# ctb/khmer

Hardware: NVIDIA B200
Metric: kmers_per_sec_countgraph_k20_N4 (higher is better)
Workload: dtype u8

## Files before the change

### include/kmgpu.h

```cpp
#ifndef KMGPU_H
#define KMGPU_H

#include <stddef.h>
#include <stdint.h>

#ifdef __cplusplus
extern "C" {
#endif

#define KMGPU_ABI_VERSION 2

enum { KMGPU_BYTE = 0, KMGPU_NIBBLE = 1, KMGPU_BIT = 2 };
enum { KMGPU_TWOBIT = 0, KMGPU_MURMUR = 1 };

#define KMGPU_CLEAN 1u

enum {
    KMGPU_OK = 0,
    KMGPU_EINVAL = 1,
    KMGPU_ENODEV = 2,
    KMGPU_ECUDA = 3,
    KMGPU_ENOMEM = 4,
    KMGPU_ENONACGT = 5,
    KMGPU_ESHAPE = 6,
// ... 95 lines not shown
int kmgpu_ipc_export(kmgpu_t* h, uint8_t* handles );
int kmgpu_ipc_attach(kmgpu_t* h, int rank, int world, const uint8_t* all_handles );
int kmgpu_ipc_detach(kmgpu_t* h);
int kmgpu_reduce_scatter_peers(kmgpu_t* h);
int kmgpu_all_gather_peers(kmgpu_t* h);
int kmgpu_reduce_replicas(kmgpu_t** replicas, int n);
int kmgpu_attach_replicas(kmgpu_t** replicas, int n);
int kmgpu_slice_range(uint64_t n_words, int world, int rank, uint64_t* w0, uint64_t* w1);

int kmgpu_first_touch_log(kmgpu_t* h, int on);
int kmgpu_first_touch_resolve(kmgpu_t* h, uint64_t* n_new_out, uint64_t* n_local_out, uint64_t* hist);

typedef struct kmgpu_shard kmgpu_shard_t;
#define KMGPU_SHARD_IPC_HANDLES 5
#define KMGPU_MAX_WORLD 16
int kmgpu_shard_create(int storage, int hash, int ksize, int n_tables, const uint64_t* full_sizes, int device,
                       int rank, int world, uint64_t max_positions_per_route, kmgpu_shard_t** out);
int kmgpu_shard_destroy(kmgpu_shard_t* s);
kmgpu_t* kmgpu_shard_local(kmgpu_shard_t* s);
int kmgpu_shard_slice(kmgpu_shard_t* s, int table, uint64_t* lo, uint64_t* hi);
int kmgpu_shard_stats(kmgpu_shard_t* s, uint64_t* n_occupied_local, uint64_t* n_unique_share, uint64_t* store_bytes);
int kmgpu_shard_ipc_export(kmgpu_shard_t* s, uint8_t* handles);
int kmgpu_shard_ipc_attach(kmgpu_shard_t* s, const uint8_t* all_handles);
int kmgpu_shard_attach_local(kmgpu_shard_t** all, int n);
int kmgpu_shard_route(kmgpu_shard_t* s, const char* seqs, const uint64_t* offsets, uint64_t n_reads, uint32_t flags,
                      uint64_t* n_kmers_out);
int kmgpu_shard_offsets(kmgpu_shard_t* s);
int kmgpu_shard_push(kmgpu_shard_t* s);
int kmgpu_shard_apply(kmgpu_shard_t* s);
int kmgpu_shard_count_new(kmgpu_shard_t* s, uint64_t* n_new_out);

int kmgpu_profile_reset(kmgpu_t* h);
int kmgpu_profile_get(kmgpu_t* h, double* ingest_kernel_ms, uint64_t* ingest_launches, uint64_t* all_launches);
int kmgpu_sync(kmgpu_t* h);
int kmgpu_timer_start(kmgpu_t* h);
int kmgpu_timer_stop(kmgpu_t* h, double* ms);

typedef struct kmgpu_hll kmgpu_hll_t;
int kmgpu_hll_create(int device, int ksize, int n_counters_log2, kmgpu_hll_t** out);
int kmgpu_hll_destroy(kmgpu_hll_t* c);
int kmgpu_hll_consume(kmgpu_hll_t* c, const char* seqs, const uint64_t* offsets, uint64_t n_reads, uint32_t flags, uint64_t* n_kmers_out);
int kmgpu_hll_get_registers(kmgpu_hll_t* c, uint8_t* out);
int kmgpu_hll_merge_registers(kmgpu_hll_t* c, const uint8_t* in, int replace);

#ifdef __cplusplus
}
#endif
#endif
```

### khmer_b200/cabi.py

```python
import ctypes as C
import os

import numpy as np

HERE = os.path.dirname(os.path.abspath(__file__))
LIB_PATH = os.path.join(HERE, "libkmgpu.so")

BYTE, NIBBLE, BIT = 0, 1, 2
TWOBIT, MURMUR = 0, 1
CLEAN = 1

u8p = C.POINTER(C.c_uint8)
u16p = C.POINTER(C.c_uint16)
u32p = C.POINTER(C.c_uint32)
u64p = C.POINTER(C.c_uint64)
f32p = C.POINTER(C.c_float)

SYMBOLS = [
    "kmgpu_last_error", "kmgpu_abi_version", "kmgpu_device_count", "kmgpu_create", "kmgpu_destroy",
    "kmgpu_set_use_bigcount", "kmgpu_get_use_bigcount", "kmgpu_consume_reads", "kmgpu_consume_packed",
    "kmgpu_batch_create", "kmgpu_batch_destroy", "kmgpu_batch_info", "kmgpu_consume_batch", "kmgpu_batch_read_medians", "kmgpu_add_hashes",
    "kmgpu_get_counts", "kmgpu_kmer_counts", "kmgpu_kmer_hashes", "kmgpu_read_medians", "kmgpu_median_at_least",
    "kmgpu_abundance_distribution", "kmgpu_trim_batch", "kmgpu_normalize_batch", "kmgpu_consume_reads_new", "kmgpu_first_touch_log",
    "kmgpu_first_touch_resolve", "kmgpu_stats", "kmgpu_set_stats", "kmgpu_shape", "kmgpu_set_ksize",
    "kmgpu_table_nbytes", "kmgpu_download_table", "kmgpu_upload_table", "kmgpu_bigcount_size",
    "kmgpu_bigcount_export", "kmgpu_bigcount_import", "kmgpu_merge", "kmgpu_recount_occupied", "kmgpu_ipc_export",
    "kmgpu_ipc_attach", "kmgpu_ipc_detach", "kmgpu_reduce_scatter_peers", "kmgpu_all_gather_peers",
    "kmgpu_reduce_replicas", "kmgpu_attach_replicas", "kmgpu_profile_reset", "kmgpu_profile_get", "kmgpu_sync", "kmgpu_reset",
    "kmgpu_timer_start", "kmgpu_timer_stop", "kmgpu_slice_range", "kmgpu_alloc_pinned", "kmgpu_free_pinned",
    "kmgpu_shard_create", "kmgpu_shard_destroy", "kmgpu_shard_local", "kmgpu_shard_slice", "kmgpu_shard_ipc_export",
    "kmgpu_shard_ipc_attach", "kmgpu_shard_attach_local", "kmgpu_shard_route", "kmgpu_shard_offsets", "kmgpu_shard_push", "kmgpu_shard_apply",
    "kmgpu_shard_count_new", "kmgpu_shard_stats", "kmgpu_hll_create", "kmgpu_hll_destroy", "kmgpu_hll_consume",
    "kmgpu_hll_get_registers", "kmgpu_hll_merge_registers",
]


class Band(C.Structure):
    _fields_ = [("lo", C.c_uint64), ("hi", C.c_uint64)]


class Mask(C.Structure):
    _fields_ = [("mask", C.c_void_p), ("threshold", C.c_uint32), ("consume_masked", C.c_int)]


class KmgpuError(RuntimeError):
    def __init__(self, code, msg):
        super().__init__("kmgpu error %d: %s" % (code, msg))
        self.code = code
        self.msg = msg


_lib = None


def lib():
    global _lib
    if _lib is None:
        if not os.path.exists(LIB_PATH):
            raise ImportError("%s is missing: build it with `python -c 'import __graft_entry__ as g; g.build()'` "
                              "(nvcc, sm_100a). There is no CPU fallback." % LIB_PATH)
        L = C.CDLL(LIB_PATH)
# ... 25 lines not shown
                                         C.c_void_p, C.c_void_p, C.c_void_p]
        L.kmgpu_median_at_least.argtypes = [C.c_void_p, C.c_void_p, C.c_void_p, C.c_uint64, C.c_uint32, C.c_uint32,
                                            C.c_void_p]
        L.kmgpu_abundance_distribution.argtypes = [C.c_void_p, C.c_void_p, C.c_void_p, C.c_void_p, C.c_uint64,
                                                   C.c_uint32, C.c_void_p]
        L.kmgpu_trim_batch.argtypes = [C.c_void_p, C.c_void_p, C.c_void_p, C.c_uint64, C.c_uint32, C.c_uint32, C.c_int, C.c_void_p]
        L.kmgpu_normalize_batch.argtypes = [C.c_void_p, C.c_void_p, C.c_void_p, C.c_uint64, C.c_uint32, C.c_void_p, C.c_uint32,
                                            C.c_void_p, u64p, u64p]
        L.kmgpu_consume_reads_new.argtypes = [C.c_void_p, C.c_void_p, C.c_void_p, C.c_uint64, C.c_uint32, C.c_void_p, u64p, u64p]
        L.kmgpu_first_touch_log.argtypes = [C.c_void_p, C.c_int]
        L.kmgpu_first_touch_resolve.argtypes = [C.c_void_p, u64p, u64p, C.c_void_p]
        L.kmgpu_stats.argtypes = [C.c_void_p, u64p, u64p]
        L.kmgpu_set_stats.argtypes = [C.c_void_p, C.c_uint64, C.c_uint64]
        L.kmgpu_shape.argtypes = [C.c_void_p, C.POINTER(C.c_int), C.POINTER(C.c_int), C.POINTER(C.c_int),
                                  C.POINTER(C.c_int), u64p]
        L.kmgpu_set_ksize.argtypes = [C.c_void_p, C.c_int]
        L.kmgpu_table_nbytes.argtypes = [C.c_void_p, C.c_int, u64p]
        L.kmgpu_download_table.argtypes = [C.c_void_p, C.c_int, C.c_void_p, C.c_uint64, C.c_uint64]
        L.kmgpu_upload_table.argtypes = [C.c_void_p, C.c_int, C.c_void_p, C.c_uint64, C.c_uint64]
        L.kmgpu_bigcount_size.argtypes = [C.c_void_p, u64p]
        L.kmgpu_bigcount_export.argtypes = [C.c_void_p, C.c_void_p, C.c_void_p, C.c_uint64]
        L.kmgpu_bigcount_import.argtypes = [C.c_void_p, C.c_void_p, C.c_void_p, C.c_uint64]
        L.kmgpu_merge.argtypes = [C.c_void_p, C.c_void_p]
        L.kmgpu_recount_occupied.argtypes = [C.c_void_p]
        L.kmgpu_ipc_export.argtypes = [C.c_void_p, C.c_void_p]
        L.kmgpu_ipc_attach.argtypes = [C.c_void_p, C.c_int, C.c_int, C.c_void_p]
        L.kmgpu_ipc_detach.argtypes = [C.c_void_p]
        L.kmgpu_reduce_scatter_peers.argtypes = [C.c_void_p]
        L.kmgpu_all_gather_peers.argtypes = [C.c_void_p]
        L.kmgpu_reduce_replicas.argtypes = [C.POINTER(C.c_void_p), C.c_int]
        L.kmgpu_attach_replicas.argtypes = [C.POINTER(C.c_void_p), C.c_int]
        L.kmgpu_profile_reset.argtypes = [C.c_void_p]
        L.kmgpu_profile_get.argtypes = [C.c_void_p, C.POINTER(C.c_double), u64p, u64p]
        L.kmgpu_sync.argtypes = [C.c_void_p]
        L.kmgpu_reset.argtypes = [C.c_void_p]
        L.kmgpu_timer_start.argtypes = [C.c_void_p]
        L.kmgpu_timer_stop.argtypes = [C.c_void_p, C.POINTER(C.c_double)]
        L.kmgpu_device_count.argtypes = [C.POINTER(C.c_int)]
        L.kmgpu_slice_range.argtypes = [C.c_uint64, C.c_int, C.c_int, u64p, u64p]
        L.kmgpu_shard_create.argtypes = [C.c_int, C.c_int, C.c_int, C.c_int, u64p, C.c_int, C.c_int, C.c_int, C.c_uint64,
                                         C.POINTER(C.c_void_p)]
        L.kmgpu_shard_destroy.argtypes = [C.c_void_p]
        L.kmgpu_shard_local.restype = C.c_void_p
        L.kmgpu_shard_local.argtypes = [C.c_void_p]
        L.kmgpu_shard_slice.argtypes = [C.c_void_p, C.c_int, u64p, u64p]
        L.kmgpu_shard_ipc_export.argtypes = [C.c_void_p, C.c_void_p]
        L.kmgpu_shard_ipc_attach.argtypes = [C.c_void_p, C.c_void_p]
        L.kmgpu_shard_attach_local.argtypes = [C.POINTER(C.c_void_p), C.c_int]
        L.kmgpu_shard_route.argtypes = [C.c_void_p, C.c_void_p, C.c_void_p, C.c_uint64, C.c_uint32, u64p]
        L.kmgpu_shard_apply.argtypes = [C.c_void_p]
        L.kmgpu_shard_offsets.argtypes = [C.c_void_p]
        L.kmgpu_shard_push.argtypes = [C.c_void_p]
        L.kmgpu_shard_count_new.argtypes = [C.c_void_p, u64p]
        L.kmgpu_shard_stats.argtypes = [C.c_void_p, u64p, u64p, u64p]
        _lib = L
    return _lib


def check(rc):
    if rc != 0:
        raise KmgpuError(rc, lib().kmgpu_last_error().decode(errors="replace"))


def device_count():
    n = C.c_int()
    rc = lib().kmgpu_device_count(C.byref(n))
# ... 291 lines not shown

    def merge(self, other):
        check(lib().kmgpu_merge(self.h, other.h))

    def recount_occupied(self):
        check(lib().kmgpu_recount_occupied(self.h))

    def ipc_export(self):
        out = np.zeros(64 * len(self.sizes), dtype=np.uint8)
        check(lib().kmgpu_ipc_export(self.h, _ptr(out)))
        return out

    def ipc_attach(self, rank, world, all_handles):
        all_handles = np.ascontiguousarray(all_handles, dtype=np.uint8)
        check(lib().kmgpu_ipc_attach(self.h, rank, world, _ptr(all_handles)))

    def ipc_detach(self):
        check(lib().kmgpu_ipc_detach(self.h))

    def reduce_scatter_peers(self):
        check(lib().kmgpu_reduce_scatter_peers(self.h))

    def all_gather_peers(self):
        check(lib().kmgpu_all_gather_peers(self.h))

    def profile_reset(self):
        check(lib().kmgpu_profile_reset(self.h))

    def profile_get(self):
        ms, a, b = C.c_double(), C.c_uint64(), C.c_uint64()
        check(lib().kmgpu_profile_get(self.h, C.byref(ms), C.byref(a), C.byref(b)))
        return ms.value, a.value, b.value

    def sync(self):
        check(lib().kmgpu_sync(self.h))

    def reset(self):
        check(lib().kmgpu_reset(self.h))

    def timer_start(self):
        check(lib().kmgpu_timer_start(self.h))

    def timer_stop(self):
        ms = C.c_double()
        check(lib().kmgpu_timer_stop(self.h, C.byref(ms)))
        return ms.value


SHARD_IPC_HANDLES = 5


class Shard:

    def __init__(self, storage, hashkind, ksize, full_sizes, rank, world, device=0, max_positions=8 << 20):
        self.full_sizes = [int(x) for x in full_sizes]
        arr = (C.c_uint64 * len(self.full_sizes))(*self.full_sizes)
        self.h = C.c_void_p()
        self.storage, self.rank, self.world, self.max_positions = storage, rank, world, max_positions
        check(lib().kmgpu_shard_create(storage, hashkind, ksize, len(self.full_sizes), arr, device, rank, world, max_positions,
                                       C.byref(self.h)))
        self.local = Sketch.__new__(Sketch)
        self.local.h = C.c_void_p(lib().kmgpu_shard_local(self.h))
        self.local.sizes = [max(hi - lo, 1) for lo, hi in (self.slice(i) for i in range(len(self.full_sizes)))]
        self.local.storage, self.local.hashkind, self.local.ksize = storage, hashkind, ksize
        self.local.close = lambda: None

# ... 84 lines not shown
```

### khmer_b200/csrc/kmgpu_api.cu

```cuda
#include <algorithm>
#include <cstdarg>
#include <cstdio>
#include <cstdlib>
#include <cstring>
#include <chrono>
#include <functional>
#include <mutex>
#include <string>
#include <unordered_map>
#include <vector>

#include "../../include/kmgpu.h"
#include "kmgpu_kernels.cuh"
#include "kmgpu_group.cuh"

using namespace kmgpu;

static thread_local std::string g_err;

static int fail(int code, const char* fmt, ...)
{
    char buf[1024];
    va_list ap;
    va_start(ap, fmt);
// ... 1016 lines not shown
    h->all_launches += 1;
    CK(cudaGetLastError());
    CK(cudaMemcpyAsync(h->h_evout.p, h->d_evout.p, n_distinct * sizeof(EvOut), cudaMemcpyDeviceToHost, st));
    CK(cudaStreamSynchronize(st));
    std::vector<EvOut> evs(h->h_evout.p, h->h_evout.p + n_distinct);
    std::sort(evs.begin(), evs.end(), [](const EvOut& a, const EvOut& b) { return a.first < b.first; });
    for (const EvOut& e : evs) big_events(h, e.hash, e.count);
    return KMGPU_OK;
}

static bool plan_buckets(const kmgpu_sketch* h, uint32_t n_pos, BucketLayout* L)
{
    if (!env_u64("KMGPU_BUCKETS", 1)) return false;
    memset(L, 0, sizeof *L);
    L->n_tables = h->nt;
    uint64_t cap = 0, total = 0;
    for (int i = 0; i < h->nt; i++) {
        if (h->sizes[i] > 0xFFFFFFFEull - 128) return false;
        uint64_t nb = (h->sizes[i] + BKT_BINS - 1) / BKT_BINS;
        if (nb > (uint64_t)BKT_MAX_BUCKETS) return false;
        L->first[i] = (uint32_t)total;
        total += nb;
        uint64_t expect = nb == 1 ? n_pos : (uint64_t)((double)n_pos * BKT_BINS / (double)h->sizes[i]) + 1;
        cap = std::max(cap, expect + expect / 4 + 2048);
    }
    L->first[h->nt] = (uint32_t)total;
    cap = std::min<uint64_t>(cap, (uint64_t)n_pos);
    if (uint64_t forced = env_u64("KMGPU_BUCKET_CAP", 0)) cap = forced;
    if (cap > 65535 || cap == 0) return false;
    L->cap = (uint32_t)cap;
    return true;
}

template <int KIND>
static void launch_apply(unsigned g, cudaStream_t st, const SketchDev& S, const BucketLayout& L, const unsigned long long* rec, const uint32_t* cur,
                         uint32_t* newbits, uint64_t* binlist, unsigned long long list_cap, Ctrl* ctrl, int want_cross, const SatBits& sb)
{
    k_apply<KIND><<<g, 1024, BKT_APPLY_SMEM, st>>>(S, L, rec, cur, newbits, binlist, list_cap, ctrl, want_cross, sb);
}

typedef std::function<int()> Between;

#include "kmgpu_group_host.inc"

static int ingest_chunk_delta(kmgpu_sketch* h, const std::vector<DeltaPass>& passes, int src, HashCfg H, const std::vector<Part>& parts, const Pred& P,
                              bool pred, const SketchDev* M, ChunkResult* res, const Between& between)
{
    cudaStream_t st = h->stream;
    uint32_t n_pos = 0;
    for (const Part& pt : parts) n_pos = std::max(n_pos, pt.pos_off + pt.in.n_pos);
    const uint64_t stride = ((uint64_t)n_pos + 7) & ~7ull;
    CKR(h->d_bins.ensure((size_t)h->nt * stride));
    uint64_t total_bins = 0, max_span = 0;
    for (int i = 0; i < h->nt; i++) total_bins += h->sizes[i];
    for (const DeltaPass& p : passes) max_span = std::max<uint64_t>(max_span, p.hi - p.lo);
    const uint64_t list_cap = std::max<uint64_t>(1, std::min<uint64_t>((uint64_t)h->nt * n_pos, total_bins));
    CKR(h->d_binlist.ensure(list_cap));
    size_t need_lanes = h->kind == BIT ? ((max_span + 127) / 128) * 8 + 8 : ((max_span + 7) & ~7ull) + 8;
    if (h->d_delta.cap < need_lanes) h->delta_zeroed = 0;
    CKR(h->d_delta.ensure(need_lanes));
    if (h->delta_zeroed < h->d_delta.cap) {
        CK(cudaMemsetAsync(h->d_delta.p, 0, h->d_delta.cap * 2, st));
        h->delta_zeroed = h->d_delta.cap;
    }
    CK(cudaMemsetAsync(h->d_ctrl, 0, sizeof(Ctrl), st));
    CK(cudaEventRecord(h->ev0, st));
    const int want_cross = h->kind == BYTE && h->use_bigcount;
    if (want_cross && !h->satbits_valid) {
        for (int i = 0; i < h->nt; i++) {
            uint64_t groups = (h->sizes[i] + 7) / 8;
            CKR(h->d_satbits[i].ensure(groups));
            k_build_satbits<<<(unsigned)std::min<uint64_t>((groups + 255) / 256, 148 * 16), 256, 0, st>>>(h->dev.tables[i], groups, h->d_satbits[i].p);
            h->all_launches += 1;
        }
        h->satbits_valid = true;
    }
    bool kmers_counted = false;
    BucketLayout BL;
    bool use_buckets = plan_buckets(h, n_pos, &BL);
    if (use_buckets) {
        if (!h->bucket_attr_set) {
            CK(cudaFuncSetAttribute(k_bucketize<BKT_TILE, BKT_PER>, cudaFuncAttributeMaxDynamicSharedMemorySize, (int)bkt_sort_smem(BKT_TILE)));
            CK(cudaFuncSetAttribute(k_apply<BYTE>, cudaFuncAttributeMaxDynamicSharedMemorySize, (int)BKT_APPLY_SMEM));
            CK(cudaFuncSetAttribute(k_apply<NIBBLE>, cudaFuncAttributeMaxDynamicSharedMemorySize, (int)BKT_APPLY_SMEM));
            CK(cudaFuncSetAttribute(k_apply<BIT>, cudaFuncAttributeMaxDynamicSharedMemorySize, (int)BKT_APPLY_SMEM));
            h->bucket_attr_set = true;
        }
        const uint32_t n_buckets = BL.first[h->nt];
        if (h->d_records.ensure((size_t)n_buckets * BL.cap) != KMGPU_OK) {
            cudaGetLastError();
            use_buckets = false;
        }
    }
    if (use_buckets) {
        const uint32_t n_buckets = BL.first[h->nt];
        CKR(h->d_cursors.ensure(n_buckets));
        const size_t nb_words = (n_pos + 31) / 32;
        CKR(h->d_newbits.ensure(nb_words));
        CK(cudaMemsetAsync(h->d_cursors.p, 0, (size_t)n_buckets * 4, st));
        CK(cudaMemsetAsync(h->d_newbits.p, 0, nb_words * 4, st));
    }
    for (const Part& pt : parts) {
        const Input& in = pt.in;
        if (pt.ready) CK(cudaStreamWaitEvent(st, pt.ready, 0));
        if (in.n_pos == 0) continue;
        uint32_t* bins = h->d_bins.p + pt.pos_off;
        const unsigned g = n_tiles(in.n_pos);
        const SketchDev& MS = M ? *M : h->dev;
        if (src == 1) launch_hashbins<TWOBIT, 1>(pred, g, st, h->dev, MS, H, P, in, bins, stride, h->d_ctrl);
        else if (H.kind == TWOBIT) launch_hashbins<TWOBIT, 0>(pred, g, st, h->dev, MS, H, P, in, bins, stride, h->d_ctrl);
        else launch_hashbins<MURMUR, 0>(pred, g, st, h->dev, MS, H, P, in, bins, stride, h->d_ctrl);
        if (use_buckets)
            k_bucketize<BKT_TILE, BKT_PER><<<dim3((in.n_pos + BKT_TILE - 1) / BKT_TILE, h->nt), BKT_TILE / BKT_PER, bkt_sort_smem(BKT_TILE), st>>>(
                bins, stride, in.n_pos, pt.pos_off, BL, h->d_records.p, h->d_cursors.p, h->d_ctrl);
        h->ingest_launches += use_buckets ? 2 : 1;
        h->all_launches += use_buckets ? 2 : 1;
    }
    if (use_buckets) {
        const uint32_t n_buckets = BL.first[h->nt];
        const size_t nb_words = (n_pos + 31) / 32;
        SatBits sb;
        memset(&sb, 0, sizeof sb);
        if (want_cross)
            for (int i = 0; i < h->nt; i++) sb.t[i] = h->d_satbits[i].p;
        if (h->kind == BYTE) launch_apply<BYTE>(n_buckets, st, h->dev, BL, h->d_records.p, h->d_cursors.p, h->d_newbits.p, h->d_binlist.p, list_cap, h->d_ctrl, want_cross, sb);
        else if (h->kind == NIBBLE) launch_apply<NIBBLE>(n_buckets, st, h->dev, BL, h->d_records.p, h->d_cursors.p, h->d_newbits.p, h->d_binlist.p, list_cap, h->d_ctrl, 0, sb);
        else launch_apply<BIT>(n_buckets, st, h->dev, BL, h->d_records.p, h->d_cursors.p, h->d_newbits.p, h->d_binlist.p, list_cap, h->d_ctrl, 0, sb);
        k_popc<<<(unsigned)std::min<size_t>((nb_words + 255) / 256, 148 * 8), 256, 0, st>>>(h->d_newbits.p, nb_words, &h->d_ctrl->n_unique);
        CK(cudaEventRecord(h->ev1, st));
        CK(cudaGetLastError());
        if (between) CKR(between());
        CKR(read_ctrl(h));
        float ms = 0;
        CK(cudaEventElapsedTime(&ms, h->ev0, h->ev1));
        h->ingest_ms += ms;
        h->ingest_launches += 2;
        h->all_launches += 2;
        Ctrl c = *h->h_ctrl;
        res->n_kmers += c.n_kmers;
        kmers_counted = true;
        if (!c.overflow) {
            if (c.n_events > list_cap) return fail(KMGPU_ECUDA, "internal: bin list overflow");
            h->n_occupied += c.n_z0;
            if (c.n_zbits) {
                h->n_unique += c.n_unique;
                res->n_new += c.n_unique;
                res->have_newbits = true;
// ... 2247 lines not shown
```

### khmer_b200/csrc/kmgpu_kernels.cuh

```cuda
#pragma once
#include "kmgpu_device.cuh"

namespace kmgpu {

struct Ctrl {
    unsigned long long n_kmers;
    unsigned long long n_z0;
    unsigned long long n_zbits;
    unsigned long long n_allsat;
    unsigned long long n_sat;
    unsigned long long n_cross;
    unsigned long long n_unique;
    unsigned long long n_events;
    unsigned long long non_acgt;
    unsigned long long n_new_t[32];
    unsigned long long pass_list_end[64];
    unsigned long long overflow;
    unsigned long long queue_overflow;
};

constexpr uint32_t F_CONSUMED = 1u << 31;
constexpr int F_MAXT = 10;
constexpr uint64_t FILTER_BITS = 1ull << 23;
constexpr uint64_t FILTER_WORDS = FILTER_BITS / 32;
// ... 1182 lines not shown
__global__ void __launch_bounds__(256)
k_pk_replay_all(const uint32_t* __restrict__ bins, uint64_t stride, int n_tables, uint32_t n_pos, PkLayout L, unsigned long long* slots,
                const uint32_t* __restrict__ filter)
{
    uint32_t p = blockIdx.x * 256u + threadIdx.x;
    if (p >= n_pos) return;
    uint32_t b[F_MAXT];
    bool act[F_MAXT];
#pragma unroll
    for (int t = 0; t < F_MAXT; t++) b[t] = t < n_tables ? __ldcs(&bins[t * stride + p]) : BIN_NONE;
    if (b[0] == BIN_NONE) return;
    const uint32_t fmask = L.filter_bits - 1, fwords = L.filter_bits >> 5;
#pragma unroll
    for (int t = 0; t < F_MAXT; t++) {
        act[t] = t < n_tables && L.mask[t] != 0;
        if (act[t] && L.use_filter) act[t] = (__ldg(&filter[t * fwords + ((b[t] & fmask) >> 5)]) >> (b[t] & 31)) & 1u;
    }
#pragma unroll
    for (int t = 0; t < F_MAXT; t++) {
        if (!act[t]) continue;
        unsigned long long* tb = slots + L.base[t];
        uint64_t s = pk_slot0(b[t], L.mask[t]);
        pk_finish(tb, L.mask[t], s, __ldcg(&tb[s]), b[t], p);
    }
}

struct SatBits {
    const uint8_t* t[F_MAXT];
};

constexpr int BKT_SHIFT = 15;
constexpr uint32_t BKT_BINS = 1u << BKT_SHIFT;
constexpr int BKT_MAX_BUCKETS = 6144;
constexpr int BKT_PER = 16;
constexpr int BKT_TILE = 16384;
constexpr size_t BKT_APPLY_SMEM = (size_t)BKT_BINS * 2 + (size_t)BKT_BINS * 4;
constexpr size_t bkt_sort_smem(int tile) { return (size_t)tile * 8 + (size_t)BKT_MAX_BUCKETS * 12; }

struct BucketLayout {
    uint32_t first[F_MAXT + 1];
    uint32_t cap;
    int n_tables;
};

template <int T, int PER>
__global__ void __launch_bounds__(T / PER, 1)
k_bucketize(const uint32_t* __restrict__ bins, uint64_t stride, uint32_t n_pos, uint32_t pos_base, BucketLayout L,
            unsigned long long* __restrict__ records, uint32_t* __restrict__ cursors, Ctrl* ctrl)
{
    constexpr int NT = T / PER;
    constexpr int BPT = (BKT_MAX_BUCKETS + NT - 1) / NT;
    extern __shared__ __align__(16) unsigned char bk_raw[];
    uint2* stage = reinterpret_cast<uint2*>(bk_raw);
    uint2* run = stage + T;
    uint32_t* hist = reinterpret_cast<uint32_t*>(run + BKT_MAX_BUCKETS);
    __shared__ uint32_t s_warp[32];
    __shared__ uint32_t s_total;
    const int t = blockIdx.y;
    const uint32_t nb = L.first[t + 1] - L.first[t];
    const uint32_t p0 = blockIdx.x * (uint32_t)T;
    const uint32_t tid = threadIdx.x;
    uint32_t bin[PER], rk[PER / 2];
    const uint32_t* src = bins + (size_t)t * stride;
#pragma unroll
    for (int j = 0; j < PER; j++) {
        uint32_t p = p0 + j * NT + tid;
        bin[j] = p < n_pos ? __ldcs(src + p) : BIN_NONE;
    }
    for (uint32_t i = tid; i < nb; i += NT) hist[i] = 0;
    __syncthreads();
#pragma unroll
    for (int j = 0; j < PER; j++) {
        uint32_t r = bin[j] != BIN_NONE ? atomicAdd(&hist[bin[j] >> BKT_SHIFT], 1u) : 0u;
        if (j & 1) rk[j >> 1] |= r << 16; else rk[j >> 1] = r;
    }
    __syncthreads();
    uint32_t c[BPT], mine = 0;
#pragma unroll
    for (int q = 0; q < BPT; q++) {
        uint32_t b = tid * BPT + q;
        c[q] = b < nb ? hist[b] : 0;
        mine += c[q];
    }
    uint32_t incl = mine;
    const uint32_t lane = tid & 31, wid = tid >> 5;
#pragma unroll
    for (int o = 1; o < 32; o <<= 1) {
        uint32_t v = __shfl_up_sync(0xffffffffu, incl, o);
        if (lane >= (uint32_t)o) incl += v;
    }
    if (lane == 31) s_warp[wid] = incl;
    __syncthreads();
    if (wid == 0) {
        uint32_t v = lane < NT / 32 ? s_warp[lane] : 0, w = v;
#pragma unroll
        for (int o = 1; o < 32; o <<= 1) {
            uint32_t u = __shfl_up_sync(0xffffffffu, w, o);
            if (lane >= (uint32_t)o) w += u;
        }
        s_warp[lane] = w - v;
        if (lane == 31) s_total = w;
    }
    __syncthreads();
    uint32_t at = s_warp[wid] + incl - mine, gbase[BPT];
#pragma unroll
    for (int q = 0; q < BPT; q++) {
        uint32_t b = tid * BPT + q;
        if (b < nb) run[b].x = at;
        gbase[q] = c[q] ? atomicAdd(&cursors[L.first[t] + b], c[q]) : 0u;
        at += c[q];
    }
    __syncthreads();
#pragma unroll
    for (int j = 0; j < PER; j++) {
        if (bin[j] == BIN_NONE) continue;
        const uint32_t b = bin[j] >> BKT_SHIFT;
        const uint32_t r = (j & 1) ? rk[j >> 1] >> 16 : rk[j >> 1] & 0xFFFFu;
        stage[run[b].x + r] = make_uint2(((uint32_t)(j * NT + tid) << BKT_SHIFT) | (bin[j] & (BKT_BINS - 1)), (b << 16) | r);
    }
#pragma unroll
    for (int q = 0; q < BPT; q++) {
        uint32_t b = tid * BPT + q;
        if (b < nb) run[b].y = gbase[q];
    }
    __syncthreads();
    const uint32_t total = s_total;
    const size_t base = (size_t)L.first[t] * L.cap;
    bool over = false;
    for (uint32_t s = tid; s < total; s += NT) {
        const uint2 m = stage[s];
        const uint32_t b = m.y >> 16, idx = run[b].y + (m.y & 0xFFFFu);
        if (idx < L.cap)
            records[base + (size_t)b * L.cap + idx] = ((unsigned long long)(pos_base + p0 + (m.x >> BKT_SHIFT)) << BKT_SHIFT) | (m.x & (BKT_BINS - 1));
        else
            over = true;
    }
    if (over) atomicExch(&ctrl->overflow, 1ull);
}

__global__ void k_popc(const uint32_t* __restrict__ words, uint64_t n, unsigned long long* out)
{
    unsigned cnt = 0;
    for (uint64_t i = blockIdx.x * (uint64_t)blockDim.x + threadIdx.x; i < n; i += (uint64_t)gridDim.x * blockDim.x) cnt += __popc(words[i]);
    cnt = __reduce_add_sync(0xffffffffu, cnt);
    if ((threadIdx.x & 31) == 0 && cnt) atomicAdd(out, (unsigned long long)cnt);
}

template <int KIND>
__global__ void __launch_bounds__(1024, 1)
k_apply(SketchDev S, BucketLayout L, const unsigned long long* __restrict__ records, const uint32_t* __restrict__ cursors,
        uint32_t* __restrict__ newbits, uint64_t* __restrict__ binlist, unsigned long long list_cap, Ctrl* ctrl, int want_cross, SatBits sb)
{
    extern __shared__ __align__(16) uint32_t ap_smem[];
    uint32_t* cnt = ap_smem;
    uint32_t* minpos = ap_smem + BKT_BINS / 2;
    if (ctrl->overflow) return;
    const uint32_t n = cursors[blockIdx.x];
    if (n == 0) return;
    int t = 0;
    uint32_t first_t = 0;
    const uint8_t* sat = nullptr;
#pragma unroll
    for (int i = 0; i < F_MAXT; i++)
        if (i < L.n_tables && blockIdx.x >= L.first[i]) {
            t = i;
            first_t = L.first[i];
// ... 390 lines not shown
```

Measured before the change: 21.68 billion.

## Restructure bucketize kernel: larger tile, compact smem staging, templated bucket scan

The bucketize kernel now uses a 32768-position tile with 1024 threads and a compact shared-memory layout: 4-byte low words plus 2-byte bucket ids instead of 8-byte staged records, and a single reused per-bucket word array replacing separate run and hist arrays. The per-bucket offset is folded into one subtraction so the scatter pass needs no rank field, and bins are re-read from global memory during the scatter instead of being kept in registers. The bucket-per-thread count is chosen at launch from the actual bucket count, and an occupancy query API is added. The intent is to cut shared-memory footprint and register pressure and to amortise per-block scan and cursor atomics over more positions. The cost is a second global read of the bins.

```diff
diff --git a/include/kmgpu.h b/include/kmgpu.h
--- a/include/kmgpu.h
+++ b/include/kmgpu.h
@@ -151,6 +151,7 @@
 
 int kmgpu_profile_reset(kmgpu_t* h);
 int kmgpu_profile_get(kmgpu_t* h, double* ingest_kernel_ms, uint64_t* ingest_launches, uint64_t* all_launches);
+int kmgpu_bucketize_occupancy(kmgpu_t* h, uint64_t n_pos, int* ctas_per_sm);
 int kmgpu_sync(kmgpu_t* h);
 int kmgpu_timer_start(kmgpu_t* h);
 int kmgpu_timer_stop(kmgpu_t* h, double* ms);
diff --git a/khmer_b200/cabi.py b/khmer_b200/cabi.py
--- a/khmer_b200/cabi.py
+++ b/khmer_b200/cabi.py
@@ -26,7 +26,7 @@
     "kmgpu_table_nbytes", "kmgpu_download_table", "kmgpu_upload_table", "kmgpu_bigcount_size",
     "kmgpu_bigcount_export", "kmgpu_bigcount_import", "kmgpu_merge", "kmgpu_recount_occupied", "kmgpu_ipc_export",
     "kmgpu_ipc_attach", "kmgpu_ipc_detach", "kmgpu_reduce_scatter_peers", "kmgpu_all_gather_peers",
-    "kmgpu_reduce_replicas", "kmgpu_attach_replicas", "kmgpu_profile_reset", "kmgpu_profile_get", "kmgpu_sync", "kmgpu_reset",
+    "kmgpu_reduce_replicas", "kmgpu_attach_replicas", "kmgpu_profile_reset", "kmgpu_profile_get", "kmgpu_bucketize_occupancy", "kmgpu_sync", "kmgpu_reset",
     "kmgpu_timer_start", "kmgpu_timer_stop", "kmgpu_slice_range", "kmgpu_alloc_pinned", "kmgpu_free_pinned",
     "kmgpu_shard_create", "kmgpu_shard_destroy", "kmgpu_shard_local", "kmgpu_shard_slice", "kmgpu_shard_ipc_export",
     "kmgpu_shard_ipc_attach", "kmgpu_shard_attach_local", "kmgpu_shard_route", "kmgpu_shard_offsets", "kmgpu_shard_push", "kmgpu_shard_apply",
@@ -118,6 +118,7 @@
         L.kmgpu_attach_replicas.argtypes = [C.POINTER(C.c_void_p), C.c_int]
         L.kmgpu_profile_reset.argtypes = [C.c_void_p]
         L.kmgpu_profile_get.argtypes = [C.c_void_p, C.POINTER(C.c_double), u64p, u64p]
+        L.kmgpu_bucketize_occupancy.argtypes = [C.c_void_p, C.c_uint64, C.POINTER(C.c_int)]
         L.kmgpu_sync.argtypes = [C.c_void_p]
         L.kmgpu_reset.argtypes = [C.c_void_p]
         L.kmgpu_timer_start.argtypes = [C.c_void_p]
@@ -475,6 +476,11 @@
         check(lib().kmgpu_profile_get(self.h, C.byref(ms), C.byref(a), C.byref(b)))
         return ms.value, a.value, b.value
 
+    def bucketize_occupancy(self, n_pos):
+        n = C.c_int()
+        check(lib().kmgpu_bucketize_occupancy(self.h, n_pos, C.byref(n)))
+        return n.value
+
     def sync(self):
         check(lib().kmgpu_sync(self.h))
 
diff --git a/khmer_b200/csrc/kmgpu_api.cu b/khmer_b200/csrc/kmgpu_api.cu
--- a/khmer_b200/csrc/kmgpu_api.cu
+++ b/khmer_b200/csrc/kmgpu_api.cu
@@ -1072,6 +1072,44 @@
     return true;
 }
 
+template <int BPT>
+static int launch_bucketize_inst(uint32_t nb_max, int n_tables, cudaStream_t st, const uint32_t* bins, uint64_t stride, uint32_t n_pos,
+                                 uint32_t pos_base, const BucketLayout& L, unsigned long long* rec, uint32_t* cur, Ctrl* ctrl, int* occupancy)
+{
+    static bool attr = false;
+    if (!attr) {
+        CK(cudaFuncSetAttribute(k_bucketize<BPT>, cudaFuncAttributeMaxDynamicSharedMemorySize, (int)bkt_smem(BKT_MAX_BUCKETS)));
+        attr = true;
+    }
+    if (occupancy) {
+        CK(cudaOccupancyMaxActiveBlocksPerMultiprocessor(occupancy, k_bucketize<BPT>, BKT_THREADS, bkt_smem(nb_max)));
+        return KMGPU_OK;
+    }
+    k_bucketize<BPT><<<dim3((n_pos + BKT_TILE - 1) / BKT_TILE, n_tables), BKT_THREADS, bkt_smem(nb_max), st>>>(bins, stride, n_pos, pos_base, L, rec,
+                                                                                                          cur, ctrl);
+    return KMGPU_OK;
+}
+
+static int launch_bucketize(const BucketLayout& L, cudaStream_t st, const uint32_t* bins, uint64_t stride, uint32_t n_pos, uint32_t pos_base,
+                            unsigned long long* rec, uint32_t* cur, Ctrl* ctrl, int* occupancy = nullptr)
+{
+    uint32_t nb_max = 0;
+    for (int i = 0; i < L.n_tables; i++) nb_max = std::max(nb_max, L.first[i + 1] - L.first[i]);
+    if (nb_max <= 3 * BKT_THREADS) return launch_bucketize_inst<3>(nb_max, L.n_tables, st, bins, stride, n_pos, pos_base, L, rec, cur, ctrl, occupancy);
+    return launch_bucketize_inst<6>(nb_max, L.n_tables, st, bins, stride, n_pos, pos_base, L, rec, cur, ctrl, occupancy);
+}
+
+extern "C" int kmgpu_bucketize_occupancy(kmgpu_t* h, uint64_t n_pos, int* ctas_per_sm)
+{
+    if (!h || !ctas_per_sm) return fail(KMGPU_EINVAL, "null argument");
+    *ctas_per_sm = 0;
+    if (n_pos == 0 || n_pos > 0xFFFFFFFFull) return fail(KMGPU_EINVAL, "n_pos must be within 1 .. 2^32 - 1");
+    BucketLayout L;
+    if (!plan_buckets(h, (uint32_t)n_pos, &L)) return KMGPU_OK;
+    CKR(set_device(h->device));
+    return launch_bucketize(L, h->stream, nullptr, 0, (uint32_t)n_pos, 0, nullptr, nullptr, nullptr, ctas_per_sm);
+}
+
 template <int KIND>
 static void launch_apply(unsigned g, cudaStream_t st, const SketchDev& S, const BucketLayout& L, const unsigned long long* rec, const uint32_t* cur,
                          uint32_t* newbits, uint64_t* binlist, unsigned long long list_cap, Ctrl* ctrl, int want_cross, const SatBits& sb)
@@ -1120,7 +1158,6 @@
     bool use_buckets = plan_buckets(h, n_pos, &BL);
     if (use_buckets) {
         if (!h->bucket_attr_set) {
-            CK(cudaFuncSetAttribute(k_bucketize<BKT_TILE, BKT_PER>, cudaFuncAttributeMaxDynamicSharedMemorySize, (int)bkt_sort_smem(BKT_TILE)));
             CK(cudaFuncSetAttribute(k_apply<BYTE>, cudaFuncAttributeMaxDynamicSharedMemorySize, (int)BKT_APPLY_SMEM));
             CK(cudaFuncSetAttribute(k_apply<NIBBLE>, cudaFuncAttributeMaxDynamicSharedMemorySize, (int)BKT_APPLY_SMEM));
             CK(cudaFuncSetAttribute(k_apply<BIT>, cudaFuncAttributeMaxDynamicSharedMemorySize, (int)BKT_APPLY_SMEM));
@@ -1150,9 +1187,7 @@
         if (src == 1) launch_hashbins<TWOBIT, 1>(pred, g, st, h->dev, MS, H, P, in, bins, stride, h->d_ctrl);
         else if (H.kind == TWOBIT) launch_hashbins<TWOBIT, 0>(pred, g, st, h->dev, MS, H, P, in, bins, stride, h->d_ctrl);
         else launch_hashbins<MURMUR, 0>(pred, g, st, h->dev, MS, H, P, in, bins, stride, h->d_ctrl);
-        if (use_buckets)
-            k_bucketize<BKT_TILE, BKT_PER><<<dim3((in.n_pos + BKT_TILE - 1) / BKT_TILE, h->nt), BKT_TILE / BKT_PER, bkt_sort_smem(BKT_TILE), st>>>(
-                bins, stride, in.n_pos, pt.pos_off, BL, h->d_records.p, h->d_cursors.p, h->d_ctrl);
+        if (use_buckets) CKR(launch_bucketize(BL, st, bins, stride, in.n_pos, pt.pos_off, h->d_records.p, h->d_cursors.p, h->d_ctrl));
         h->ingest_launches += use_buckets ? 2 : 1;
         h->all_launches += use_buckets ? 2 : 1;
     }
diff --git a/khmer_b200/csrc/kmgpu_kernels.cuh b/khmer_b200/csrc/kmgpu_kernels.cuh
--- a/khmer_b200/csrc/kmgpu_kernels.cuh
+++ b/khmer_b200/csrc/kmgpu_kernels.cuh
@@ -1238,10 +1238,12 @@
 constexpr int BKT_SHIFT = 15;
 constexpr uint32_t BKT_BINS = 1u << BKT_SHIFT;
 constexpr int BKT_MAX_BUCKETS = 6144;
-constexpr int BKT_PER = 16;
-constexpr int BKT_TILE = 16384;
 constexpr size_t BKT_APPLY_SMEM = (size_t)BKT_BINS * 2 + (size_t)BKT_BINS * 4;
-constexpr size_t bkt_sort_smem(int tile) { return (size_t)tile * 8 + (size_t)BKT_MAX_BUCKETS * 12; }
+constexpr int BKT_TILE = 32768;
+constexpr int BKT_THREADS = 1024;
+constexpr size_t bkt_smem(uint32_t nb) { return (size_t)BKT_TILE * 6 + (size_t)nb * 4; }
+static_assert(bkt_smem(BKT_MAX_BUCKETS) <= 227 * 1024, "k_bucketize shared memory");
+static_assert(BKT_MAX_BUCKETS <= 6 * BKT_THREADS, "the widest k_bucketize scan covers 6 buckets per thread");
 
 struct BucketLayout {
     uint32_t first[F_MAXT + 1];
@@ -1249,95 +1251,105 @@
     int n_tables;
 };
 
-template <int T, int PER>
-__global__ void __launch_bounds__(T / PER, 1)
+template <int BPT>
+__global__ void __launch_bounds__(BKT_THREADS, 1)
 k_bucketize(const uint32_t* __restrict__ bins, uint64_t stride, uint32_t n_pos, uint32_t pos_base, BucketLayout L,
             unsigned long long* __restrict__ records, uint32_t* __restrict__ cursors, Ctrl* ctrl)
 {
-    constexpr int NT = T / PER;
-    constexpr int BPT = (BKT_MAX_BUCKETS + NT - 1) / NT;
+    constexpr int T = BKT_TILE, NT = BKT_THREADS, PER = T / NT;
+    static_assert(T <= 32768, "positions in the tile and ranks are held in 15 and 16 bits");
     extern __shared__ __align__(16) unsigned char bk_raw[];
-    uint2* stage = reinterpret_cast<uint2*>(bk_raw);
-    uint2* run = stage + T;
-    uint32_t* hist = reinterpret_cast<uint32_t*>(run + BKT_MAX_BUCKETS);
-    __shared__ uint32_t s_warp[32];
-    __shared__ uint32_t s_total;
+    uint32_t* low = reinterpret_cast<uint32_t*>(bk_raw);
+    uint16_t* bkt = reinterpret_cast<uint16_t*>(low + T);
+    uint32_t* word = reinterpret_cast<uint32_t*>(bkt + T);
+    __shared__ uint32_t s_warp[NT / 32];
     const int t = blockIdx.y;
     const uint32_t nb = L.first[t + 1] - L.first[t];
     const uint32_t p0 = blockIdx.x * (uint32_t)T;
+    const uint32_t n = min(n_pos - p0, (uint32_t)T);
     const uint32_t tid = threadIdx.x;
+    const uint32_t* src = bins + (size_t)t * stride + p0;
     uint32_t bin[PER], rk[PER / 2];
-    const uint32_t* src = bins + (size_t)t * stride;
 #pragma unroll
     for (int j = 0; j < PER; j++) {
-        uint32_t p = p0 + j * NT + tid;
-        bin[j] = p < n_pos ? __ldcs(src + p) : BIN_NONE;
-    }
-    for (uint32_t i = tid; i < nb; i += NT) hist[i] = 0;
+        const uint32_t p = j * NT + tid;
+        bin[j] = p < n ? src[p] : BIN_NONE;
+    }
+    for (uint32_t i = tid; i < nb; i += NT) word[i] = 0;
     __syncthreads();
 #pragma unroll
     for (int j = 0; j < PER; j++) {
-        uint32_t r = bin[j] != BIN_NONE ? atomicAdd(&hist[bin[j] >> BKT_SHIFT], 1u) : 0u;
+        const uint32_t r = bin[j] != BIN_NONE ? atomicAdd(&word[bin[j] >> BKT_SHIFT], 1u) : 0u;
         if (j & 1) rk[j >> 1] |= r << 16; else rk[j >> 1] = r;
     }
     __syncthreads();
     uint32_t c[BPT], mine = 0;
 #pragma unroll
     for (int q = 0; q < BPT; q++) {
-        uint32_t b = tid * BPT + q;
-        c[q] = b < nb ? hist[b] : 0;
+        const uint32_t b = tid * BPT + q;
+        c[q] = b < nb ? word[b] : 0;
         mine += c[q];
     }
     uint32_t incl = mine;
     const uint32_t lane = tid & 31, wid = tid >> 5;
 #pragma unroll
     for (int o = 1; o < 32; o <<= 1) {
-        uint32_t v = __shfl_up_sync(0xffffffffu, incl, o);
+        const uint32_t v = __shfl_up_sync(0xffffffffu, incl, o);
         if (lane >= (uint32_t)o) incl += v;
     }
     if (lane == 31) s_warp[wid] = incl;
     __syncthreads();
-    if (wid == 0) {
-        uint32_t v = lane < NT / 32 ? s_warp[lane] : 0, w = v;
-#pragma unroll
-        for (int o = 1; o < 32; o <<= 1) {
-            uint32_t u = __shfl_up_sync(0xffffffffu, w, o);
-            if (lane >= (uint32_t)o) w += u;
-        }
-        s_warp[lane] = w - v;
-        if (lane == 31) s_total = w;
-    }
-    __syncthreads();
-    uint32_t at = s_warp[wid] + incl - mine, gbase[BPT];
+    uint32_t before = 0, total = 0;
+#pragma unroll
+    for (int w = 0; w < NT / 32; w++) {
+        const uint32_t v = s_warp[w];
+        before += (uint32_t)w < wid ? v : 0u;
+        total += v;
+    }
+    uint32_t* cur = cursors + L.first[t] + tid * BPT;
+    uint32_t gbase[BPT];
+#pragma unroll
+    for (int q = 0; q < BPT; q++) gbase[q] = c[q] ? atomicAdd(cur + q, c[q]) : 0u;
+    uint32_t at = before + incl - mine;
 #pragma unroll
     for (int q = 0; q < BPT; q++) {
-        uint32_t b = tid * BPT + q;
-        if (b < nb) run[b].x = at;
-        gbase[q] = c[q] ? atomicAdd(&cursors[L.first[t] + b], c[q]) : 0u;
+        const uint32_t b = tid * BPT + q;
+        if (b < nb) word[b] = at;
         at += c[q];
     }
     __syncthreads();
-#pragma unroll
-    for (int j = 0; j < PER; j++) {
-        if (bin[j] == BIN_NONE) continue;
-        const uint32_t b = bin[j] >> BKT_SHIFT;
-        const uint32_t r = (j & 1) ? rk[j >> 1] >> 16 : rk[j >> 1] & 0xFFFFu;
-        stage[run[b].x + r] = make_uint2(((uint32_t)(j * NT + tid) << BKT_SHIFT) | (bin[j] & (BKT_BINS - 1)), (b << 16) | r);
-    }
+    constexpr int RB = 8;
+#pragma unroll
+    for (int j0 = 0; j0 < PER; j0 += RB) {
+        uint32_t v[RB];
+#pragma unroll
+        for (int i = 0; i < RB; i++) {
+            const uint32_t p = (j0 + i) * NT + tid;
+            v[i] = p < n ? __ldcs(src + p) : BIN_NONE;
+        }
+#pragma unroll
+        for (int i = 0; i < RB; i++) {
+            if (v[i] == BIN_NONE) continue;
+            const int j = j0 + i;
+            const uint32_t b = v[i] >> BKT_SHIFT;
+            const uint32_t slot = word[b] + ((j & 1) ? rk[j >> 1] >> 16 : rk[j >> 1] & 0xFFFFu);
+            low[slot] = ((uint32_t)(j * NT + tid) << BKT_SHIFT) | (v[i] & (BKT_BINS - 1));
+            bkt[slot] = (uint16_t)b;
+        }
+    }
+    __syncthreads();
 #pragma unroll
     for (int q = 0; q < BPT; q++) {
-        uint32_t b = tid * BPT + q;
-        if (b < nb) run[b].y = gbase[q];
-    }
-    __syncthreads();
-    const uint32_t total = s_total;
+        const uint32_t b = tid * BPT + q;
+        if (b < nb) word[b] = gbase[q] - word[b];
+    }
+    __syncthreads();
     const size_t base = (size_t)L.first[t] * L.cap;
     bool over = false;
     for (uint32_t s = tid; s < total; s += NT) {
-        const uint2 m = stage[s];
-        const uint32_t b = m.y >> 16, idx = run[b].y + (m.y & 0xFFFFu);
+        const uint32_t m = low[s], b = bkt[s], idx = word[b] + s;
         if (idx < L.cap)
-            records[base + (size_t)b * L.cap + idx] = ((unsigned long long)(pos_base + p0 + (m.x >> BKT_SHIFT)) << BKT_SHIFT) | (m.x & (BKT_BINS - 1));
+            records[base + (size_t)b * L.cap + idx] = ((unsigned long long)(pos_base + p0 + (m >> BKT_SHIFT)) << BKT_SHIFT) | (m & (BKT_BINS - 1));
         else
             over = true;
     }
```

Result: no change. 21.88 billion (median of 6 runs) (+0.9%).

## Rewrite bucketize with larger tiles, packed 16-bit counters and compact smem staging

Applied to the files above, without the earlier changes.

Reworks the bucketize kernel to use 32K-position tiles with 1024 threads, two buckets packed per 32-bit shared counter, and 4-byte staging entries instead of 8-byte ones. Run heads are located through a bitmap plus per-word run index and a bias table, so each record's destination comes from a popcount. A smaller-bucket template variant is chosen when every table has at most 4096 buckets. The aim is to cut shared memory per element and per-tile global cursor atomics, in exchange for more complex index math and a second atomic pass for scatter ranks.

```diff
diff --git a/khmer_b200/csrc/kmgpu_api.cu b/khmer_b200/csrc/kmgpu_api.cu
--- a/khmer_b200/csrc/kmgpu_api.cu
+++ b/khmer_b200/csrc/kmgpu_api.cu
@@ -1120,7 +1120,10 @@
     bool use_buckets = plan_buckets(h, n_pos, &BL);
     if (use_buckets) {
         if (!h->bucket_attr_set) {
-            CK(cudaFuncSetAttribute(k_bucketize<BKT_TILE, BKT_PER>, cudaFuncAttributeMaxDynamicSharedMemorySize, (int)bkt_sort_smem(BKT_TILE)));
+            CK(cudaFuncSetAttribute(k_bucketize<BKT_TILE, BKT_SMALL_BUCKETS>, cudaFuncAttributeMaxDynamicSharedMemorySize,
+                                    (int)bkt_sort_smem(BKT_TILE, BKT_SMALL_BUCKETS)));
+            CK(cudaFuncSetAttribute(k_bucketize<BKT_TILE, BKT_MAX_BUCKETS>, cudaFuncAttributeMaxDynamicSharedMemorySize,
+                                    (int)bkt_sort_smem(BKT_TILE, BKT_MAX_BUCKETS)));
             CK(cudaFuncSetAttribute(k_apply<BYTE>, cudaFuncAttributeMaxDynamicSharedMemorySize, (int)BKT_APPLY_SMEM));
             CK(cudaFuncSetAttribute(k_apply<NIBBLE>, cudaFuncAttributeMaxDynamicSharedMemorySize, (int)BKT_APPLY_SMEM));
             CK(cudaFuncSetAttribute(k_apply<BIT>, cudaFuncAttributeMaxDynamicSharedMemorySize, (int)BKT_APPLY_SMEM));
@@ -1132,8 +1135,10 @@
             use_buckets = false;
         }
     }
+    bool small_buckets = true;
     if (use_buckets) {
         const uint32_t n_buckets = BL.first[h->nt];
+        for (int i = 0; i < h->nt; i++) small_buckets &= BL.first[i + 1] - BL.first[i] <= (uint32_t)BKT_SMALL_BUCKETS;
         CKR(h->d_cursors.ensure(n_buckets));
         const size_t nb_words = (n_pos + 31) / 32;
         CKR(h->d_newbits.ensure(nb_words));
@@ -1150,9 +1155,15 @@
         if (src == 1) launch_hashbins<TWOBIT, 1>(pred, g, st, h->dev, MS, H, P, in, bins, stride, h->d_ctrl);
         else if (H.kind == TWOBIT) launch_hashbins<TWOBIT, 0>(pred, g, st, h->dev, MS, H, P, in, bins, stride, h->d_ctrl);
         else launch_hashbins<MURMUR, 0>(pred, g, st, h->dev, MS, H, P, in, bins, stride, h->d_ctrl);
-        if (use_buckets)
-            k_bucketize<BKT_TILE, BKT_PER><<<dim3((in.n_pos + BKT_TILE - 1) / BKT_TILE, h->nt), BKT_TILE / BKT_PER, bkt_sort_smem(BKT_TILE), st>>>(
-                bins, stride, in.n_pos, pt.pos_off, BL, h->d_records.p, h->d_cursors.p, h->d_ctrl);
+        if (use_buckets) {
+            const dim3 grid((in.n_pos + BKT_TILE - 1) / BKT_TILE, h->nt);
+            if (small_buckets)
+                k_bucketize<BKT_TILE, BKT_SMALL_BUCKETS><<<grid, BKT_THREADS, bkt_sort_smem(BKT_TILE, BKT_SMALL_BUCKETS), st>>>(
+                    bins, stride, in.n_pos, pt.pos_off, BL, h->d_records.p, h->d_cursors.p, h->d_ctrl);
+            else
+                k_bucketize<BKT_TILE, BKT_MAX_BUCKETS><<<grid, BKT_THREADS, bkt_sort_smem(BKT_TILE, BKT_MAX_BUCKETS), st>>>(
+                    bins, stride, in.n_pos, pt.pos_off, BL, h->d_records.p, h->d_cursors.p, h->d_ctrl);
+        }
         h->ingest_launches += use_buckets ? 2 : 1;
         h->all_launches += use_buckets ? 2 : 1;
     }
diff --git a/khmer_b200/csrc/kmgpu_kernels.cuh b/khmer_b200/csrc/kmgpu_kernels.cuh
--- a/khmer_b200/csrc/kmgpu_kernels.cuh
+++ b/khmer_b200/csrc/kmgpu_kernels.cuh
@@ -1238,10 +1238,11 @@
 constexpr int BKT_SHIFT = 15;
 constexpr uint32_t BKT_BINS = 1u << BKT_SHIFT;
 constexpr int BKT_MAX_BUCKETS = 6144;
-constexpr int BKT_PER = 16;
-constexpr int BKT_TILE = 16384;
+constexpr int BKT_SMALL_BUCKETS = 4096;
+constexpr int BKT_TILE = 32768;
+constexpr int BKT_THREADS = 1024;
 constexpr size_t BKT_APPLY_SMEM = (size_t)BKT_BINS * 2 + (size_t)BKT_BINS * 4;
-constexpr size_t bkt_sort_smem(int tile) { return (size_t)tile * 8 + (size_t)BKT_MAX_BUCKETS * 12; }
+constexpr size_t bkt_sort_smem(int tile, int maxb) { return (size_t)tile * 4 + (size_t)tile / 32 * 8 + (size_t)maxb * 4 + (size_t)maxb * 2; }
 
 struct BucketLayout {
     uint32_t first[F_MAXT + 1];
@@ -1249,47 +1250,50 @@
     int n_tables;
 };
 
-template <int T, int PER>
-__global__ void __launch_bounds__(T / PER, 1)
+template <int T, int MAXB>
+__global__ void __launch_bounds__(BKT_THREADS, 1)
 k_bucketize(const uint32_t* __restrict__ bins, uint64_t stride, uint32_t n_pos, uint32_t pos_base, BucketLayout L,
             unsigned long long* __restrict__ records, uint32_t* __restrict__ cursors, Ctrl* ctrl)
 {
-    constexpr int NT = T / PER;
-    constexpr int BPT = (BKT_MAX_BUCKETS + NT - 1) / NT;
-    extern __shared__ __align__(16) unsigned char bk_raw[];
-    uint2* stage = reinterpret_cast<uint2*>(bk_raw);
-    uint2* run = stage + T;
-    uint32_t* hist = reinterpret_cast<uint32_t*>(run + BKT_MAX_BUCKETS);
-    __shared__ uint32_t s_warp[32];
-    __shared__ uint32_t s_total;
+    constexpr int NT = BKT_THREADS, PER = T / NT;
+    constexpr int WPT = MAXB / 2 / NT;
+    constexpr int HW = T / 32;
+    static_assert(T % NT == 0 && HW % NT == 0 && MAXB % (2 * NT) == 0 && T <= 32768 && MAXB <= 8192, "k_bucketize shape");
+    extern __shared__ __align__(16) uint32_t bk_smem[];
+    uint32_t* stage = bk_smem;
+    uint32_t* head = stage + T;
+    uint32_t* before = head + HW;
+    uint32_t* bias = before + HW;
+    uint32_t* ctr = bias + MAXB;
+    __shared__ uint32_t s_warp[NT / 32];
     const int t = blockIdx.y;
-    const uint32_t nb = L.first[t + 1] - L.first[t];
     const uint32_t p0 = blockIdx.x * (uint32_t)T;
-    const uint32_t tid = threadIdx.x;
-    uint32_t bin[PER], rk[PER / 2];
+    const uint32_t tid = threadIdx.x, lane = tid & 31, wid = tid >> 5;
     const uint32_t* src = bins + (size_t)t * stride;
+    uint32_t bin[PER];
 #pragma unroll
     for (int j = 0; j < PER; j++) {
         uint32_t p = p0 + j * NT + tid;
         bin[j] = p < n_pos ? __ldcs(src + p) : BIN_NONE;
     }
-    for (uint32_t i = tid; i < nb; i += NT) hist[i] = 0;
-    __syncthreads();
-#pragma unroll
-    for (int j = 0; j < PER; j++) {
-        uint32_t r = bin[j] != BIN_NONE ? atomicAdd(&hist[bin[j] >> BKT_SHIFT], 1u) : 0u;
-        if (j & 1) rk[j >> 1] |= r << 16; else rk[j >> 1] = r;
-    }
-    __syncthreads();
-    uint32_t c[BPT], mine = 0;
-#pragma unroll
-    for (int q = 0; q < BPT; q++) {
-        uint32_t b = tid * BPT + q;
-        c[q] = b < nb ? hist[b] : 0;
-        mine += c[q];
+#pragma unroll
+    for (int q = 0; q < WPT; q++) ctr[q * NT + tid] = 0;
+#pragma unroll
+    for (int q = 0; q < HW / NT; q++) head[q * NT + tid] = 0;
+#pragma unroll
+    for (int j = 0; j < PER; j++) stage[j * NT + tid] = bin[j];
+    __syncthreads();
+#pragma unroll
+    for (int j = 0; j < PER; j++)
+        if (bin[j] != BIN_NONE) atomicAdd(&ctr[bin[j] >> (BKT_SHIFT + 1)], (bin[j] >> BKT_SHIFT & 1) ? 0x10000u : 1u);
+    __syncthreads();
+    uint32_t mine = 0;
+#pragma unroll
+    for (int q = 0; q < WPT; q++) {
+        const uint32_t h = ctr[tid * WPT + q], lo = h & 0xFFFFu, hi = h >> 16;
+        mine += ((uint32_t)(lo != 0) + (uint32_t)(hi != 0)) << 16 | (lo + hi);
     }
     uint32_t incl = mine;
-    const uint32_t lane = tid & 31, wid = tid >> 5;
 #pragma unroll
     for (int o = 1; o < 32; o <<= 1) {
         uint32_t v = __shfl_up_sync(0xffffffffu, incl, o);
@@ -1297,47 +1301,59 @@
     }
     if (lane == 31) s_warp[wid] = incl;
     __syncthreads();
-    if (wid == 0) {
-        uint32_t v = lane < NT / 32 ? s_warp[lane] : 0, w = v;
-#pragma unroll
-        for (int o = 1; o < 32; o <<= 1) {
-            uint32_t u = __shfl_up_sync(0xffffffffu, w, o);
-            if (lane >= (uint32_t)o) w += u;
-        }
-        s_warp[lane] = w - v;
-        if (lane == 31) s_total = w;
-    }
-    __syncthreads();
-    uint32_t at = s_warp[wid] + incl - mine, gbase[BPT];
-#pragma unroll
-    for (int q = 0; q < BPT; q++) {
-        uint32_t b = tid * BPT + q;
-        if (b < nb) run[b].x = at;
-        gbase[q] = c[q] ? atomicAdd(&cursors[L.first[t] + b], c[q]) : 0u;
-        at += c[q];
-    }
+    uint32_t at = __reduce_add_sync(0xffffffffu, lane < wid ? s_warp[lane] : 0u) + incl - mine;
+    const uint32_t total = __reduce_add_sync(0xffffffffu, lane < NT / 32 ? s_warp[lane] : 0u) & 0xFFFFu;
+    const uint32_t run0 = at >> 16;
+    uint32_t gb[2 * WPT], nonempty = 0;
+#pragma unroll
+    for (int q = 0; q < WPT; q++) {
+        const uint32_t h = ctr[tid * WPT + q];
+        uint32_t offs = 0;
+#pragma unroll
+        for (int e = 0; e < 2; e++) {
+            const uint32_t c = e ? h >> 16 : h & 0xFFFFu, b = (tid * WPT + q) * 2 + e, off = at & 0xFFFFu, r = at >> 16;
+            offs |= off << (16 * e);
+            gb[2 * q + e] = 0;
+            if (!c) continue;
+            nonempty |= 1u << (2 * q + e);
+            gb[2 * q + e] = atomicAdd(&cursors[L.first[t] + b], c);
+            atomicOr(&head[off >> 5], 1u << (off & 31));
+            bias[r] = b << 18 | ((0u - off) & 0x3FFFFu);
+            for (uint32_t w = (off + 31) >> 5; w << 5 < off + c; w++) before[w] = r + (off < w << 5);
+            at += 1u << 16 | c;
+        }
+        ctr[tid * WPT + q] = offs;
+    }
+#pragma unroll
+    for (int j = 0; j < PER; j++) bin[j] = stage[j * NT + tid];
     __syncthreads();
 #pragma unroll
     for (int j = 0; j < PER; j++) {
         if (bin[j] == BIN_NONE) continue;
-        const uint32_t b = bin[j] >> BKT_SHIFT;
-        const uint32_t r = (j & 1) ? rk[j >> 1] >> 16 : rk[j >> 1] & 0xFFFFu;
-        stage[run[b].x + r] = make_uint2(((uint32_t)(j * NT + tid) << BKT_SHIFT) | (bin[j] & (BKT_BINS - 1)), (b << 16) | r);
-    }
-#pragma unroll
-    for (int q = 0; q < BPT; q++) {
-        uint32_t b = tid * BPT + q;
-        if (b < nb) run[b].y = gbase[q];
-    }
-    __syncthreads();
-    const uint32_t total = s_total;
+        const uint32_t hi = bin[j] >> BKT_SHIFT & 1;
+        const uint32_t s = atomicAdd(&ctr[bin[j] >> (BKT_SHIFT + 1)], hi ? 0x10000u : 1u) >> (16 * hi) & 0xFFFFu;
+        stage[s] = (uint32_t)(j * NT + tid) << BKT_SHIFT | (bin[j] & (BKT_BINS - 1));
+    }
+    uint32_t r = run0;
+#pragma unroll
+    for (int i = 0; i < 2 * WPT; i++) {
+        if (!(nonempty >> i & 1)) continue;
+        const uint32_t w = bias[r];
+        bias[r] = (w & ~0x3FFFFu) | ((w + min(gb[i], L.cap)) & 0x3FFFFu);
+        r++;
+    }
+    __syncthreads();
     const size_t base = (size_t)L.first[t] * L.cap;
     bool over = false;
-    for (uint32_t s = tid; s < total; s += NT) {
-        const uint2 m = stage[s];
-        const uint32_t b = m.y >> 16, idx = run[b].y + (m.y & 0xFFFFu);
+#pragma unroll
+    for (int j = 0; j < PER; j++) {
+        const uint32_t s = j * NT + tid;
+        if (s >= total) break;
+        const uint32_t m = stage[s], hw = head[s >> 5] & (0xFFFFFFFFu >> (31 - (s & 31)));
+        const uint32_t br = bias[before[s >> 5] + __popc(hw) - 1];
+        const uint32_t idx = s + (uint32_t)((int32_t)(br << 14) >> 14);
         if (idx < L.cap)
-            records[base + (size_t)b * L.cap + idx] = ((unsigned long long)(pos_base + p0 + (m.x >> BKT_SHIFT)) << BKT_SHIFT) | (m.x & (BKT_BINS - 1));
+            records[base + (size_t)(br >> 18) * L.cap + idx] = ((unsigned long long)(pos_base + p0 + (m >> BKT_SHIFT)) << BKT_SHIFT) | (m & (BKT_BINS - 1));
         else
             over = true;
     }
```

After: 21.83 billion before, 23.44 billion after, median of 6. 7.4% higher.
